# Immortalqx/pi-slam-fusion

Measured on AMD Instinct MI355X. Metric: keyframes/sec fused (4000x3000 -> 256^2 tiles, 5-band), higher is better.
Workload: dtype f32; 1 GPU; cfg-2/cfg-A: 4000x3000 BGR8 keyframes, serpentine sortie, Map2D.Scale=1, 5-band Laplacian, CV_32FC3 (ForceFloat=1) pyramids, frames resident in HBM; frames_per_rank=2646, sortie_frames_before_timing=20, lookahead=48, rendered_rank0=2666, culled_tiles_rank0=490117

## Files before the change

pi-slam-fusion_amd/__init__.py:

```python
import ctypes as C
import os
import subprocess

import numpy as np

_HERE = os.path.dirname(os.path.abspath(__file__))
LIB_PATH = os.environ.get("PF_LIB") or os.path.join(_HERE, "libpifusion.so")
ELE_PIXELS = 256

NoType, TypeCPU, TypeGPU, TypeMultiBandCPU, TypeRender = 0, 1, 2, 3, 4
PF_8UC3, PF_8UC4, PF_16SC3, PF_32FC3 = 16, 24, 19, 21


def host_array(shape, dtype=np.uint8):
    n = int(np.prod(shape)) * np.dtype(dtype).itemsize
    p = lib().pf_host_alloc(n)
    if not p:
        raise MemoryError("pf_host_alloc(%d)" % n)
    buf = (C.c_uint8 * n).from_address(p)
    a = np.frombuffer(buf, dtype=dtype).reshape(shape)
    import weakref
    weakref.finalize(buf, lib().pf_host_free, p)
    return a

# ... 827 lines not shown
    def render_stats(self):
        o = (C.c_double * 4)()
        lib().pf_render_stats(self._h, o)
        return {"frames_with_pixels": int(o[0]), "level0_px": o[1], "owned_px": o[2], "tiles_held": int(o[3])}

    def timers(self):
        cap = 16
        names = (C.c_char_p * cap)(); calls = (C.c_longlong * cap)(); mean = (C.c_double * cap)(); mn = (C.c_double * cap)(); mx = (C.c_double * cap)()
        k = lib().pf_timer_read(self._h, cap, names, calls, mean, mn, mx)
        return {names[i].decode(): {"calls": calls[i], "mean_s": mean[i], "min_s": mn[i], "max_s": mx[i]} for i in range(k)}

    def timer_reset(self):
        lib().pf_timer_reset(self._h)

    def set_cull(self, on):
        lib().pf_set_cull(self._h, 1 if on else 0)

    def next_homography(self, M0):
        if not hasattr(lib(), "pf_debug_next_homography"):
            raise RuntimeError("pf_debug_next_homography: only the experiments library has it (PF_LIB=.../libpifusion_exp.so)")
        a = np.ascontiguousarray(M0, dtype=np.float64).reshape(9)
        lib().pf_debug_next_homography(self._h, a.ctypes.data_as(C.POINTER(C.c_double)))

    def debug_tile_store(self, slab_slots, fail_from=0, fail_count=0):
        if not hasattr(lib(), "pf_debug_tile_store"):
            raise RuntimeError("pf_debug_tile_store: only the experiments library has it (PF_LIB=.../libpifusion_exp.so)")
        lib().pf_debug_tile_store(self._h, int(slab_slots), int(fail_from), int(fail_count))

    def debug_fail_workspace(self, n):
        if not hasattr(lib(), "pf_debug_fail_workspace"):
            raise RuntimeError("pf_debug_fail_workspace: only the experiments library has it (PF_LIB=.../libpifusion_exp.so)")
# ... 24 lines not shown
```

pi-slam-fusion_amd/csrc/c_api.cpp:

```cpp
#include "dist.hpp"
#include "jpeg_device.hpp"
#include "webtiles_plan.hpp"
#include "state_file.hpp"
#include <cerrno>
#include <map>
#include <string>
#include <sys/stat.h>
#include <cstdlib>
#include <cmath>
#include <cstdio>
#include <cstring>
#include <algorithm>
#include <vector>
#include <mutex>
#include <new>

using pf::FusionMap;

struct pf_map {
    FusionMap impl;
    pf::JpegDevice jpeg;
    pf_map(int t, bool th, const pf_options& o) : impl(t, th, o) {}
    ~pf_map() { if (impl.ok() && impl.use_device()) impl.sync(); }
};
// ... 49 lines not shown
}

void pf_destroy(pf_map* m) { delete m; }
const char* pf_last_error(void) { return pf::last_error(); }

int pf_prepare(pf_map* m, const double plane[7], const double cam[6], int n, const pf_image* imgs, const double* poses7)
{ return m && m->impl.prepare(plane, cam, n, imgs, poses7); }

int pf_feed(pf_map* m, const pf_image* img, const double pose[7]) { return m && m->impl.feed(img, pose, false); }
int pf_feed_device(pf_map* m, const pf_image* img, const double pose[7]) { return m && m->impl.feed(img, pose, true); }
int pf_debug_phase_stamps(unsigned long long* out, int cap_blocks) { return pf::read_phase_stamps(out, cap_blocks); }
void pf_debug_form_counts(long long out[8]) { if (out) pf::read_form_counts(out); }
void pf_debug_admission_counts(long long out[8]) { if (out) pf::read_admission_counts(out); }
long long pf_debug_compact_launches(void) { return pf::read_compact_launches(); }
int pf_debug_render_log(pf_map* m, long long* out, int cap) { return m ? m->impl.render_log(out, cap) : 0; }
void pf_set_cull(pf_map* m, int on) { if (m) m->impl.set_cull(on != 0); }
long long pf_debug_culled_cells(pf_map* m) { return m ? m->impl.culled_cells() : 0; }
double pf_debug_level0_exact_px(pf_map* m) { return m ? m->impl.level0_exact_px() : 0; }
long long pf_debug_culled_tiles(pf_map* m) { return m ? m->impl.culled_tiles() : 0; }
int pf_debug_select_counts(unsigned long long* out, int reset) { return out ? pf::read_select_counts(out, reset) : 0; }
long pf_debug_read_last_frame(pf_map* m, void* out, size_t cap) { return m ? m->impl.read_back_last_frame(out, cap) : -1; }
#if PF_EXPERIMENTS
void pf_debug_next_homography(pf_map* m, const double M0[9]) { if (m && M0) m->impl.debug_next_homography(M0); }
void pf_debug_tile_store(pf_map* m, int slab_slots, int fail_from, int fail_count) { if (m) m->impl.debug_tile_store(slab_slots, fail_from, fail_count); }
void pf_debug_fail_workspace(pf_map* m, int n) { if (m) m->impl.debug_fail_workspace(n); }
#endif
unsigned pf_queue_size(pf_map* m) { return m ? m->impl.queue_size() : 0; }
int pf_sync(pf_map* m) { return m && m->impl.sync(); }
int pf_save(pf_map* m, const char* filename) { return m && filename && m->impl.save(filename); }
int pf_save_tiff(pf_map* m, const char* filename, int quality, int force_bigtiff) { return m && filename && m->impl.save_tiff(filename, quality, force_bigtiff != 0); }
int pf_save_tiff_masked(pf_map* m, const char* filename, int quality, int force_bigtiff) { return m && filename && m->impl.save_tiff_masked(filename, quality, force_bigtiff != 0); }
// ... 614 lines not shown
```

pi-slam-fusion_amd/csrc/frame_plan.hpp:

```cpp
#pragma once
#include "plan_limits.hpp"
#include <algorithm>
#include <cmath>
#include <cstdint>
#include <cstring>
#include <vector>

namespace pf {

struct Win { int x0, x1, y0, y1; };


struct CullMargins { double px = 2.0, w = 1e-5; int sub = 4; };

inline bool cull_frame_ok(const double M[9], int crows, int ccols)
{
    const double xs[2] = { -600.0, ccols + 600.0 }, ys[2] = { -600.0, crows + 600.0 };
    int sign = 0;
    for (int i = 0; i < 4; i++) {
        const double x = xs[i & 1], y = ys[i >> 1], W = M[6] * x + M[7] * y + M[8];
        if (!(std::fabs(W) > 1e-12) || !std::isfinite(W)) return false;
        const int sg = W > 0 ? 1 : -1;
        if (sign && sg != sign) return false;
        sign = sg;
// ... 1 lines not shown
    }
    return true;
}

inline float stored_bound(float wlb, bool single_band)
{
    const float gap = single_band ? 3.2f / 254.f : 0.f, floor_w = single_band ? 6.f / 254.f : 0.f;
    return wlb > floor_w ? wlb - gap : 0.f;
}

struct TileCull {
    unsigned out;
    int nraise; int q[16]; float w[16];
};

struct Lattice {
    bool all = false; int nx = 0, ny = 0, dil = 1, cols = 0, rows = 0; double xc = 0, yc = 0, dis_max = 1, inv_dis_max = 1, M[9] = {};
    CullMargins mg;
    std::vector<double> sx, sy, d; std::vector<unsigned char> in;
    std::vector<double> pair_d; std::vector<unsigned char> pair_in; bool paired = false;

    void map_canvas(const double Minv[9], int crows, int ccols, int cols_, int rows_, int dil_, bool map_all, const CullMargins& m)
    {
        all = map_all; mg = m; paired = false;
        dil = dil_;
        nx = ccols / 64 + 2 * dil + 1; ny = crows / 64 + 2 * dil + 1;
        const size_t n = (size_t)nx * ny;
        sx.resize(n); sy.resize(n); d.resize(n); in.assign(n, 2);
        xc = (double)(cols_ / 2); yc = (double)(rows_ / 2); dis_max = std::sqrt(xc * xc + yc * yc);
        inv_dis_max = 1.0 / dis_max;
        cols = cols_; rows = rows_;
        for (int i = 0; i < 9; i++) M[i] = Minv[i];
        if (!map_all) return;
        const double cmax = cols - 2.0, rmax = rows - 2.0;
        for (int m_ = 0; m_ < ny; m_++) {
            const double y = 64.0 * (m_ - dil), n0 = M[1] * y + M[2], n1 = M[4] * y + M[5], w0 = M[7] * y + M[8];
            double* __restrict__ psx = sx.data() + (size_t)m_ * nx; double* __restrict__ psy = sy.data() + (size_t)m_ * nx;
            double* __restrict__ pd = d.data() + (size_t)m_ * nx; unsigned char* __restrict__ pin = in.data() + (size_t)m_ * nx;
            for (int k = 0; k < nx; k++) {
                const double x = 64.0 * (k - dil), iw = 1.0 / (M[6] * x + w0);
                const double px = (M[0] * x + n0) * iw, py = (M[3] * x + n1) * iw, dx = px - xc, dy = py - yc;
                psx[k] = px; psy[k] = py; pd[k] = dx * dx + dy * dy;
            }
            for (int k = 0; k < nx; k++) pin[k] = (unsigned char)((psx[k] >= 1.0) & (psx[k] <= cmax) & (psy[k] >= 1.0) & (psy[k] <= rmax));
        }
    }

    size_t point(int k, int m)
    {
        const size_t o = (size_t)m * nx + k;
        if (in[o] == 2) {
            const double x = 64.0 * (k - dil), y = 64.0 * (m - dil), iw = 1.0 / (M[6] * x + M[7] * y + M[8]);
            const double px = (M[0] * x + M[1] * y + M[2]) * iw, py = (M[3] * x + M[4] * y + M[5]) * iw;
            sx[o] = px; sy[o] = py;
            const double dx = px - xc, dy = py - yc;
            d[o] = dx * dx + dy * dy;
            in[o] = px >= 1.0 && px <= cols - 2.0 && py >= 1.0 && py <= rows - 2.0;
        }
        return o;
    }
// ... 9 lines not shown
            const double far2 = std::max(std::max(d2[0], d2[1]), std::max(d2[2], d2[3]));
            const double tw = weight_type == 0 ? (1.0 - mw - (double)wlb) * dis_max - mpx : 1e300;
            if ((in[c[0]] & in[c[1]] & in[c[2]] & in[c[3]]) == 1 && tw > 0 && far2 < tw * tw * (1.0 + 1e-9)) {
                const double dfar = std::sqrt(far2) + mpx;
                double w = 1.0 - dfar * inv_dis_max;
                if (weight_type != 0) w = w > 0 ? w * w : 0.0;
                w -= mw;
                if (w > 2e-5) *wmin = (float)w;
            }
        }
        if (!want_out || !(wlb > 2e-5f)) return false;
        double g = (double)wlb - mw;
        if (weight_type != 0) g = std::sqrt(g);
        const double T = mpx + dis_max * (1.0 - g), T2 = T * T;
        if (d2[0] <= T2 || d2[1] <= T2 || d2[2] <= T2 || d2[3] <= T2) return false;
        bool pos = true, neg = true; double dnear2 = 1e300;
        for (int i = 0; i < 4; i++) {
            const size_t a = c[i], b = c[(i + 1) & 3];
            const double ex = sx[b] - sx[a], ey = sy[b] - sy[a], px = xc - sx[a], py = yc - sy[a];
            const double cr = ex * py - ey * px;
            pos = pos && cr >= 0; neg = neg && cr <= 0;
            const double e2 = ex * ex + ey * ey, dot = px * ex + py * ey;
            if (dot > 0 && dot < e2) dnear2 = std::min(dnear2, cr * cr / e2);
        }
        if (pos || neg) return false;
        return dnear2 > T2;
    }

    void raise_bounds(int x, int y, int weight_type, float wlb[16])
    {
// ... 47 lines not shown
        if (ask) {
            float wl = wlb[0];
            for (int q = 1; q < S * S; q++) wl = std::min(wl, wlb[q]);
            tile_out = cell_out(4 * x, 4 * y, 4, weight_type, stored_bound(wl, single_band), true, nullptr);
        }
        if (tile_out && pre_raised) c.out = 0xffffu;
        else for (int q = 0; q < S * S; q++) {
            const int qx = q % S, qy = q / S;
            float wmin = 0.f;
            if (cell_out(4 * x + span * qx, 4 * y + span * qy, span, weight_type, stored_bound(wlb[q], single_band), ask && !tile_out, pre_raised ? nullptr : &wmin) || tile_out)
                c.out |= S == 4 ? 1u << q : 0x33u << (8 * qy + 2 * qx);
            if (wmin > wlb[q]) { c.q[c.nraise] = q; c.w[c.nraise++] = wmin; }
        }
        if (fresh && c.out != 0xffffu) c.out = 0;
    }
};

inline void clampw(int lo, int hi, int n, int& o0, int& o1) { o0 = std::max(lo, 0); o1 = std::min(hi, n); }
inline int lv_lo(int p, int i) { return p >> i; }
inline int lv_hi(int p, int i) { return (p + (1 << i) - 1) >> i; }

inline void need_windows(const Win& box, int L, int crows, int ccols, Win N[kMaxLevels])
{
    for (int i = L; i >= 0; i--) {
        int x0 = lv_lo(box.x0, i), x1 = lv_hi(box.x1, i), y0 = lv_lo(box.y0, i), y1 = lv_hi(box.y1, i);
        if (i > 0) { x0 -= 1; x1 += 1; y0 -= 1; y1 += 1; }
        if (i < L) {
            x0 = std::min(x0, 2 * N[i + 1].x0 - 2); x1 = std::max(x1, 2 * N[i + 1].x1 + 1);
            y0 = std::min(y0, 2 * N[i + 1].y0 - 2); y1 = std::max(y1, 2 * N[i + 1].y1 + 1);
        }
        clampw(x0, x1, ccols >> i, N[i].x0, N[i].x1);
        clampw(y0, y1, crows >> i, N[i].y0, N[i].y1);
    }
}

typedef unsigned __int128 u128;
inline u128 col_mask(int x0, int x1) { return (x1 - x0 >= 127 ? ~(u128)0 : (((u128)1 << (x1 - x0 + 1)) - 1)) << x0; }

struct CellList {
    struct Cell { int cx, cy, x0, y0, x1, y1; };
    Cell c[64]; int n = 0; bool overflow = false;
    void add(int cx, int cy, int x0, int y0, int x1, int y1)
    {
        if (overflow) return;
        int k = n - 1;
        while (k >= 0 && !(c[k].cx == cx && c[k].cy == cy)) k--;
        if (k < 0) {
            if (n == 64) overflow = true;
            else c[n++] = Cell{ cx, cy, x0, y0, x1, y1 };
        } else {
            Cell& e = c[k];
            e.x0 = std::min(e.x0, x0); e.y0 = std::min(e.y0, y0); e.x1 = std::max(e.x1, x1); e.y1 = std::max(e.y1, y1);
// ... 174 lines not shown
```

pi-slam-fusion_amd/csrc/fusion_map.cpp:

```cpp
#include "fusion_map.hpp"
#include "map_internal.hpp"
#include "env.hpp"
#include "warp_index.hpp"
#include <algorithm>
#include <cmath>
#include <cstdio>
#include <cstdlib>
#include <cstring>

namespace pf {

FusionMap::FusionMap(int type, bool thread, const pf_options& opt) : opt_(opt), thread_(thread)
{
    single_band_ = (type == PF_TYPE_CPU || type == PF_TYPE_GPU);
    const int lim = (int)std::ceil(std::log((double)kElePixels) / std::log(2.0));
    band_num_ = std::min(opt_.band_number, lim);
    if (band_num_ < 0) band_num_ = 0;
    if (single_band_) band_num_ = 0;
    lay_ = make_layout(band_num_, opt_.force_float != 0);
    if (single_band_) { lay_.f32 = 0; lay_.lap_off[0] = 0; lay_.w_off[0] = 0; lay_.slot_bytes = kElePixels * kElePixels * 4; }
    store_.configure(lay_.slot_bytes);
    if (opt_.max_queue <= 0) opt_.max_queue = 20;
    table_in_args_ = exp_env("PF_TABLE_COPY") == nullptr;
    if (opt_.shard_count < 1) opt_.shard_count = 1;
// ... 159 lines not shown
        p.lat.map_canvas(w.Minv, w.crows, w.ccols, f.cols, f.rows, single_band_ ? 0 : ((2 << w.L) - 2 + 63) / 64, map_all, cull_margins_);
        if (lookahead_ok()) {
            if (!tiles_pool_.empty()) { p.tiles = std::move(tiles_pool_.back()); tiles_pool_.pop_back(); }
            if (!reserve_frame_workspace(w) || !pre_raise(w, p.tiles)) {
                if (p.lat.sx.capacity() && lat_pool_.size() < 8) lat_pool_.push_back(std::move(p.lat));
                if (p.tiles.capacity() && tiles_pool_.size() < 8) tiles_pool_.push_back(std::move(p.tiles));
                pending_.pop_back();
                release_slot(f);
                keyframe_lost();
                return false;
            }
            p.pre_raised = true;
            since_drain_++;
            keep = std::min<size_t>((size_t)opt_.lookahead, 2 * (size_t)since_drain_ / 3);
        }
    }
    while (pending_.size() > keep)
        if (!render_front()) return false;
    return true;
}

bool FusionMap::pre_raise(FrameWork& w, std::vector<Tile*>& tiles)
{
    tiles.assign((size_t)w.tx * w.ty, nullptr);
    const bool sharded = opt_.shard_count > 1;
    for (int y = 0; y < w.ty; y++)
        for (int x = 0; x < w.tx; x++) {
            const int sx = w.xminInt + x + off_x_, sy = w.yminInt + y + off_y_;
            if (sharded && tile_owner(opt_.shard_count, opt_.shard_block, sx, sy) != opt_.shard_rank) continue;
            Tile* t = store_.get_or_create(sx, sy);
// ... 13 lines not shown
    slots_[f.slot].queued = false;
}

bool FusionMap::drain()
{
    since_drain_ = 0;
    if (pending_.empty()) return true;
    if (!set_device()) return false;
    bool ok = true;
    while (!pending_.empty()) ok = render_front() && ok;
    return ok;
}

bool FusionMap::render_front()
{
    const bool ok = render_front_stages();
    if (!ok) keyframe_lost();
    return ok;
}

bool FusionMap::render_front_stages()
{
    struct Pop {
        FusionMap* m;
        ~Pop() {
            PendingFrame& p = m->pending_.front();
            if (p.lat.sx.capacity() && m->lat_pool_.size() < 8) m->lat_pool_.push_back(std::move(p.lat));
            if (p.tiles.capacity() && m->tiles_pool_.size() < 8) m->tiles_pool_.push_back(std::move(p.tiles));
            m->pending_.pop_front();
        }
    } pop{ this };
    PendingFrame& p = pending_.front();
    const QueuedFrame f = p.f;
    struct Held { FusionMap* m; const QueuedFrame& f; bool done = false; ~Held() { if (!done) m->release_slot(f); } } held{ this, f };
    FrameWork& w = fw_;
    w.reset();
    std::memcpy(w.pts, p.pts, sizeof(p.pts));
    w.xminInt = p.sx0 - off_x_; w.yminInt = p.sy0 - off_y_; w.xmaxInt = w.xminInt + p.tx; w.ymaxInt = w.yminInt + p.ty;
    w.tx = p.tx; w.ty = p.ty; w.L = band_num_; w.crows = w.ty * kElePixels; w.ccols = w.tx * kElePixels;
    std::memcpy(w.M0, p.M0, sizeof(p.M0)); std::memcpy(w.Minv, p.Minv, sizeof(p.Minv));
    w.cull = p.cull;
    w.pre_raised = p.pre_raised;
    w.tiles_known = p.tiles.size() == (size_t)p.tx * p.ty ? p.tiles.data() : nullptr;
    if (w.pre_raised && !w.tiles_known) { set_error("render_front: a keyframe admitted without its tiles"); return false; }
    w.src = f.ext ? f.ext : slots_[f.slot].dev;
    w.lat = &p.lat;
    Section sec_apply(this, T_APPLY);
    if (!build_tile_table(f, w)) return false;
    if (w.bx0 >= w.bx1) {
        for (auto& r : w.raise) r.t->wlb[r.q] = std::max(r.t->wlb[r.q], r.w);
        for (Tile* t : w.culled) t->changed = true;
        if (w.owned_all) n_rendered_++;
        log_rendered(f);
        return true;
    }
    px_owned_ += (double)w.owned * kElePixels * kElePixels;
    n_with_pixels_++;
// ... 63 lines not shown
    const bool sharded = w.sharded;
    const bool cull = w.cull;
    const bool lookahead = cull && lookahead_ok();
    if (cull) w.raise.reserve((size_t)tx * ty * cull_margins_.sub * cull_margins_.sub);
    const int B = opt_.shard_block;
    static const int bc_env = exp_env_int("PF_CULL_CELL", 0);
    const int Bc = sharded ? B : (bc_env > 0 ? bc_env : 8);
    table_tmp_.resize((size_t)tx * ty);
    w.touched.reserve((size_t)tx * ty);
    w.bx0 = tx; w.bx1 = 0; w.by0 = ty; w.by1 = 0;
    w.pb = Win{ 1 << 30, 0, 1 << 30, 0 };
    auto add_rect = [&](int sx, int sy, int x0, int y0, int x1, int y1) {
        w.pb.x0 = std::min(w.pb.x0, x0); w.pb.x1 = std::max(w.pb.x1, x1); w.pb.y0 = std::min(w.pb.y0, y0); w.pb.y1 = std::max(w.pb.y1, y1);
        if (sharded || cull) w.cells.add(floordiv(sx, Bc), floordiv(sy, Bc), x0, y0, x1, y1);
    };
    for (int y = 0; y < ty; y++) {
        const int sy = w.yminInt + y + off_y_;
        for (int x = 0; x < tx; x++) {
            const int sx = w.xminInt + x + off_x_;
            uint64_t ent = 0;
            Tile* known = w.tiles_known ? w.tiles_known[(size_t)y * tx + x] : nullptr;
            if (known || ((!sharded || tile_owner(opt_.shard_count, B, sx, sy) == opt_.shard_rank) && !w.tiles_known)) {
                Tile* t = known ? known : store_.get_or_create(sx, sy);
                if (!t) return false;
                w.owned_all++;
                unsigned out = 0;
                if (cull) {
                    TileCull c;
                    w.lat->tile_cull(x, y, t->wlb, t->fresh, lookahead, w.pre_raised, opt_.weight_type, single_band_, c);
                    out = c.out;
                    for (int k = 0; k < c.nraise; k++) w.raise.push_back(FrameWork::Raise{ t, c.q[k], c.w[k] });
                    if (out == 0xffffu && t->fresh) {
                        w.culled_any = true; table_tmp_[(size_t)y * tx + x] = 0; n_culled_tiles_++;
                        continue;
                    }
                    if (out == 0xffffu) {
                        w.culled_any = true; table_tmp_[(size_t)y * tx + x] = 0; n_culled_tiles_++; w.culled.push_back(t);
                        continue;
                    }
                    if (out) { w.culled_any = true; n_culled_cells_ += __builtin_popcount(out); }
                }
                if ((uint64_t)(uintptr_t)t->base >> 48) { set_error("tile slot address above 2^48: the table entry has no room for the cell flags"); return false; }
                ent = (uint64_t)(uintptr_t)t->base | (t->fresh ? 1u : 0u) | ((uint64_t)out << 48);
                w.touched.push_back(t);
                w.owned++;
                w.bx0 = std::min(w.bx0, x); w.bx1 = std::max(w.bx1, x + 1); w.by0 = std::min(w.by0, y); w.by1 = std::max(w.by1, y + 1);
                if (!out) add_rect(sx, sy, x * kElePixels, y * kElePixels, (x + 1) * kElePixels, (y + 1) * kElePixels);
                else
                    for (int r = 0; r < 4; r++) {
                        const unsigned in = ~(out >> (4 * r)) & 15u;
                        if (!in) continue;
                        const int c0 = __builtin_ctz(in), c1 = 32 - __builtin_clz(in);
                        add_rect(sx, sy, x * kElePixels + 64 * c0, y * kElePixels + 64 * r, x * kElePixels + 64 * c1, y * kElePixels + 64 * r + 64);
                    }
            }
            table_tmp_[(size_t)y * tx + x] = ent;
        }
    }
    return true;
}

bool FusionMap::reserve_frame_workspace(FrameWork& w)
{
    const int L = w.L, tx = w.tx, ty = w.ty;
    const size_t es = lay_.f32 ? 4 : 2;
    const bool fused = opt_.fused != 0 && L >= 1;
    const size_t pxb = level_px_bytes(lay_.f32 != 0);
    bool grow = false;
    for (int i = 0; i <= L; i++) {
        const size_t n = (size_t)(w.crows >> i) * (w.ccols >> i);
        if (single_band_) continue;
        if (fused) { if (i >= 1 && i < L && (gw_[i].cap < n * pxb || gw2_[i].cap < n * pxb)) grow = true; }
        else if (g_[i].cap < n * 3 * es || wgt_[i].cap < n * 4) grow = true;
    }
// ... 350 lines not shown
```

pi-slam-fusion_amd/csrc/fusion_map.hpp:

```cpp
#pragma once
#include "../../include/pifusion.h"
#include "geometry.hpp"
#include "kernels.hpp"
#include "map_support.hpp"
#include "dist_plan.hpp"
#include "frame_plan.hpp"
#include "env.hpp"
#include "image_io.hpp"
#include "jpeg_encode.hpp"
#include "tiff_pyramid.hpp"
#include "webtiles.hpp"
#include "merge.hpp"
#include "undistort.hpp"
#include "undistort_plan.hpp"
#include <hip/hip_runtime.h>
#include <condition_variable>
#include <cstdio>
#include <cstdlib>
#include <cstring>
#include <deque>
#include <functional>
#include <mutex>
#include <string>
#include <thread>
// ... 73 lines not shown
    void list_tiles(std::vector<TileRec>& out);
    bool pack_strips(const std::vector<StripReq>& reqs, void* dev_out);
    bool export_tiles(const std::vector<std::pair<int, int>>& tiles, void* dev_out);
    bool blend_tiles(const std::vector<std::pair<int, int>>& tiles, const void* const* halo9, uint8_t* bgr);
    bool reject_mismatched_frame(const pf_image* desc);
    bool frame_needs(const double pose7[7], std::vector<unsigned char>& rank_needs);
    int  stage_frame(const pf_image* desc, bool upload_host, void** dev, size_t* bytes);
    bool feed_staged(int slot, const pf_image* desc, const double pose7[7]);
    void release_staged(int slot) { std::lock_guard<std::mutex> q(qmu_); if (slot >= 0 && slot < (int)slots_.size()) slots_[slot].queued = false; }
    hipStream_t stream() const { return stream_; }
    int  device() const { return device_; }
    bool use_device() { return set_device(); }
    bool single_band() const { return single_band_; }
    bool map_update_inputs(int ix, int iy, double plane7[7], double mn[2], double* ele, int* x, int* y);
    long long culled_tiles() { Drained l(*this); return n_culled_tiles_; }
    void set_cull(bool on) { Drained l(*this); cull_on_ = on; }
    long long culled_cells() { Drained l(*this); return n_culled_cells_; }
    int  render_log(long long* out, int cap);
    double level0_exact_px() const { return px_level0_exact_; }
#if PF_EXPERIMENTS
    void debug_next_homography(const double M0[9]) { std::lock_guard<std::mutex> l(mu_); next_M0_.emplace_back(); std::memcpy(next_M0_.back().m, M0, sizeof(double) * 9); }
    void debug_tile_store(int slab_slots, int fail_from, int fail_count) { std::lock_guard<std::mutex> l(mu_); store_.debug_limits(slab_slots, fail_from, fail_count); }
    void debug_fail_workspace(int n) { std::lock_guard<std::mutex> l(mu_); dbg_fail_workspace_ = n; }
#endif
    bool high_quality() const { return opt_.high_quality_show != 0 && !single_band_; }

    int  num_levels() const { return band_num_ + 1; }
    int  pyramid_type() const { return single_band_ ? PF_8UC4 : (lay_.f32 ? PF_32FC3 : PF_16SC3); }
    bool grid(int dims[4], double geo[6]);
    int  tile_count();
    int  tile_coords(int* xy, int cap);
// ... 110 lines not shown

    struct PipeFrame { bool valid = false; int ring = 0, tx = 0, crows = 0, ccols = 0; Win C[kMaxLevels]; double bytes[kMaxLevels], bytes_run[kMaxLevels];
                       int nrect[kMaxLevels]; BlockRect rect[kMaxLevels][kMaxRects];
                       uint32_t need_bits[kMaxLevels][kNeedWords]; int need_n[kMaxLevels] = {};
                       const uint64_t* table_args = nullptr; int table_n = 0; };
    PipeFrame pipe_[kMaxLevels];
    struct FrameWork {
        double pts[8]; int xminInt, yminInt, xmaxInt, ymaxInt;
        int tx, ty, L, crows, ccols; double M0[9], Minv[9];
        const uint8_t* src;
        bool sharded, cull, culled_any; Lattice* lat;
        bool pre_raised;
        Tile* const* tiles_known;
        struct Raise { Tile* t; int q; float w; };
        std::vector<Raise> raise; std::vector<Tile*> culled, touched;
        CellList cells;
        int bx0, bx1, by0, by1, owned, owned_all;
        Win pb;
        LevelPlan plan;
        int ring; bool table_args; const uint64_t* dtab;
        WarpArgs a;
        void reset() {
            raise.clear(); culled.clear(); touched.clear();
            culled_any = cells.overflow = false; cells.n = 0; owned = owned_all = 0; plan.reset();
            src = nullptr; ring = 0; table_args = false; dtab = nullptr; sharded = cull = pre_raised = false; tiles_known = nullptr; lat = nullptr;
        }
    };
    FrameWork fw_;
    struct PendingFrame {
        QueuedFrame f;
        double pts[8]; int sx0, sy0, tx, ty;
        double M0[9], Minv[9];
        bool cull;
        Lattice lat;
        bool pre_raised = false;
        std::vector<Tile*> tiles;
    };
    std::deque<PendingFrame> pending_;
    unsigned since_drain_ = 0;
    std::vector<Lattice> lat_pool_;
    std::vector<std::vector<Tile*>> tiles_pool_;
    bool lookahead_ok() const { return opt_.lookahead > 0 && (single_band_ || (opt_.fused == 1 && band_num_ >= 1)) && cull_on_; }
    bool render_front();
    bool render_front_stages();
    bool drain();
    void release_slot(const QueuedFrame& f);
    bool pre_raise(FrameWork& w, std::vector<Tile*>& tiles);
    void keyframe_lost() { n_failed_++; fail_pending_ = true; fail_msg_ = last_error(); }
    long long n_failed_ = 0;
    bool fail_pending_ = false;
    std::string fail_msg_;
#if PF_EXPERIMENTS
    int dbg_fail_workspace_ = 0;
#endif
    int  frame_canvas(const QueuedFrame& f, FrameWork& w);
    bool build_tile_table(const QueuedFrame& f, FrameWork& w);
    bool reserve_frame_workspace(FrameWork& w);
    bool place_table(FrameWork& w);
    void warp_args(const QueuedFrame& f, FrameWork& w);
    void plan_fused_levels(FrameWork& w);
    bool launch_single_band(const QueuedFrame& f, FrameWork& w);
    bool launch_fused_pipeline(const QueuedFrame& f, FrameWork& w);
// ... 63 lines not shown
```

pi-slam-fusion_amd/csrc/map_feed.cpp:

```cpp
#include "fusion_map.hpp"
#include "map_internal.hpp"
#include "warp_index.hpp"
#include <cmath>
#include <cstdio>
#include <cstring>
#include <new>

namespace pf {

static void print_frame_mismatch() { std::fprintf(stderr, "MultiBandMap2DCPU::renderFrame: frame.first.cols!=p->_camera.w||frame.first.rows!=p->_camera.h||frame.first.type()!=CV_8UC3\n"); }

bool FusionMap::prepare(const double plane7[7], const double cam[6], int n, const pf_image* imgs, const double* poses7)
{
    if (!init_ok_) { set_error("prepare: no device"); return false; }
    if (n == 0 || !poses7 || cam[0] <= 0 || cam[1] <= 0 || cam[2] == 0 || cam[3] == 0) {
        std::fprintf(stderr, "Map2D::prepare:Not valid prepare!\n");
        return false;
    }
    Camera c{ cam[0], cam[1], cam[2], cam[3], cam[4], cam[5], 1. / cam[2], 1. / cam[3] };
    const Pose plane = pose_from7(plane7), pinv = inverse(plane);
    double mx[3] = { -1e10, -1e10, -1e10 }, mn[3] = { 1e10, 1e10, 1e10 };
    std::vector<Pose> local(n);
    for (int i = 0; i < n; i++) {
        local[i] = mul(pinv, pose_from7(poses7 + 7 * i));
// ... 23 lines not shown
    const int h = (int)std::ceil((mx[1] - mn[1]) / ele_size);
    mx[0] = mn[0] + ele_size * w;
    mx[1] = mn[1] + ele_size * h;

    {
        std::unique_lock<std::mutex> q(qmu_);
        for (auto& f : queue_) if (f.slot >= 0) slots_[f.slot].queued = false;
        queue_.clear();
        idle_cv_.wait(q, [this] { return !worker_busy_; });
    }
    std::lock_guard<std::mutex> l(mu_);
    if (!set_device()) return false;
    if (valid_) (void)drain();
    for (auto& p : pending_) release_slot(p.f);
    pending_.clear();
    HIP_OK(sync_all());
    DevBuf und_table; long long und_uncovered = 0;
    if (und_set_ && !build_undistort_table(und_cam_, c, und_table, &und_uncovered)) return false;
    if (und_set_) { und_table_ = std::move(und_table); und_uncovered_ = und_uncovered; }
    store_.clear();
    plane_ = plane; plane_inv_ = pinv; cam_ = c;
    length_pixel_ = length_pixel; length_pixel_inv_ = 1. / length_pixel;
    ele_size_ = ele_size; ele_size_inv_ = 1. / ele_size;
    std::memcpy(min_, mn, sizeof(mn)); std::memcpy(max_, mx, sizeof(mx)); std::memcpy(min0_, mn, sizeof(mn));
    w_ = w; h_ = h; off_x_ = off_y_ = 0;
    valid_ = true;
    if (thread_ && imgs) {
        for (int i = 0; i < n; i++) {
            if (!imgs[i].data) continue;
            if (frame_mismatch(imgs[i].type, imgs[i].cols, imgs[i].rows)) { print_frame_mismatch(); continue; }
// ... 339 lines not shown
```

pi-slam-fusion_amd/csrc/map_merge.cpp:

```cpp
#include "fusion_map.hpp"
#include "map_internal.hpp"
#include "state_file.hpp"
#include <algorithm>
#include <cmath>
#include <cstdio>
#include <cstring>

namespace pf {

void FusionMap::wait_worker_idle()
{
    if (!thread_) return;
    std::unique_lock<std::mutex> q(qmu_);
    idle_cv_.wait(q, [this] { return queue_.empty() && !worker_busy_; });
}

bool FusionMap::merge_compatible(const char* who, bool single, int pyr, int bands, int weight_type, const double plane7[7], const double cam6[6],
                                 const double min0[3], double ele_size, double length_pixel)
{
    const char* why = nullptr;
    double mine7[7]; std::memcpy(mine7, plane_.t, 24); std::memcpy(mine7 + 3, plane_.q, 32);
    if (single != single_band_) why = "map types differ";
    else if (pyr != pyramid_type()) why = "pyramid types differ";
    else if (bands != band_num_) why = "band numbers differ";
// ... 4 lines not shown
        why = "the maps were prepared differently (tile coordinates are not one frame)";
    if (why) { set_error(std::string(who) + ": " + why); return false; }
    return true;
}

void FusionMap::grow_to(int sx0, int sy0, int sx1, int sy1)
{
    const Win r{ sx0 - off_x_, sx1 - off_x_, sy0 - off_y_, sy1 - off_y_ };
    if (r.x0 < 0 || r.y0 < 0 || r.x1 > w_ || r.y1 > h_) { Section sec(this, T_SPREAD); spread_tiles(r); }
}

bool FusionMap::merge_items(const std::vector<MergeItem>& items)
{
    last_merge_[0] = (double)items.size(); last_merge_[1] = last_merge_[2] = 0; last_merge_[3] = -1; last_merge_[4] = (double)lay_.slot_bytes;
    if (items.empty()) return true;
    size_t missing = 0;
    for (auto& it : items) missing += store_.find(it.ix, it.iy) == nullptr;
    if (missing && !store_.reserve(missing)) return false;
    std::vector<Tile*> tiles(items.size());
    for (size_t i = 0; i < items.size(); i++)
        if (!(tiles[i] = store_.get_or_create(items[i].ix, items[i].iy))) return false;
    if (!settle()) return false;
    std::vector<MergePair> pairs(items.size());
    size_t n_fresh = 0;
    for (size_t i = 0; i < items.size(); i++) {
        pairs[i] = MergePair{ (uint64_t)(uintptr_t)tiles[i]->base, (uint64_t)(uintptr_t)items[i].src, tiles[i]->fresh ? 1u : 0u, 0u };
        n_fresh += tiles[i]->fresh;
    }
    if (!merge_table_.reserve(pairs.size() * sizeof(MergePair))) return false;
    unsigned long long* won = nullptr;
// ... 212 lines not shown
    if ((h.map_type == sf::kTypeSingleBand) != single_band_ || h.pyramid_type != pyramid_type() || h.band_number != band_num_ || h.weight_type != opt_.weight_type) {
        set_error("load_state: the map's options (type, pyramid type, band number, weight type) are not the file's");
        return false;
    }
    {
        std::unique_lock<std::mutex> q(qmu_);
        for (auto& fr : queue_) if (fr.slot >= 0) slots_[fr.slot].queued = false;
        queue_.clear();
        idle_cv_.wait(q, [this] { return !worker_busy_; });
    }
    std::lock_guard<std::mutex> l(mu_);
    if (!set_device()) return false;
    if (valid_) (void)drain();
    for (auto& p : pending_) release_slot(p.f);
    pending_.clear();
    HIP_OK(sync_all());
    store_.clear();
    und_set_ = false; und_table_.release(); und_uncovered_ = 0;
    plane_ = pose_from7(h.plane); plane_inv_ = inverse(plane_);
    cam_ = Camera{ h.cam[0], h.cam[1], h.cam[2], h.cam[3], h.cam[4], h.cam[5], 1. / h.cam[2], 1. / h.cam[3] };
    length_pixel_ = h.length_pixel; length_pixel_inv_ = 1. / h.length_pixel;
    ele_size_ = h.ele_size; ele_size_inv_ = 1. / h.ele_size;
    std::memcpy(min_, h.min, 24); std::memcpy(max_, h.max, 24); std::memcpy(min0_, h.min0, 24);
    w_ = h.w; h_ = h.h; off_x_ = h.off_x; off_y_ = h.off_y;
    valid_ = true;
    return merge_records(f, &h, &heads);
}

}
```

pi-slam-fusion_amd/csrc/map_output.cpp:

```cpp
#include "fusion_map.hpp"
#include "map_internal.hpp"
#include "env.hpp"
#include <algorithm>
#include <cstdlib>
#include <cstring>
#include <thread>

namespace pf {

bool FusionMap::grid(int dims[4], double geo[6])
{
    std::lock_guard<std::mutex> l(mu_);
    if (!valid_) return false;
    dims[0] = w_; dims[1] = h_; dims[2] = off_x_; dims[3] = off_y_;
    geo[0] = min_[0]; geo[1] = min_[1]; geo[2] = max_[0]; geo[3] = max_[1]; geo[4] = ele_size_; geo[5] = length_pixel_;
    return true;
}

bool FusionMap::map_update_inputs(int ix, int iy, double plane7[7], double mn[2], double* ele, int* x, int* y)
{
    Drained l(*this);
    if (!valid_) return false;
    Tile* t = store_.find(ix, iy);
    if (!t || t->fresh) return false;
// ... 63 lines not shown
    Drained l(*this);
    if (!init_ok_ || !set_device()) return false;
    Tile* t = store_.find(ix, iy);
    if (!t || t->fresh) return false;
    HIP_OK(hipMemcpyAsync(dev_out, t->base, lay_.slot_bytes, hipMemcpyDeviceToDevice, stream_));
    HIP_OK(sync_all());
    return true;
}

bool FusionMap::tile_import(int ix, int iy, const void* dev_in)
{
    Drained l(*this);
    if (!init_ok_ || !valid_ || !set_device()) return false;
    Tile* t = store_.get_or_create(ix, iy);
    if (!t) return false;
    HIP_OK(hipMemcpyAsync(t->base, dev_in, lay_.slot_bytes, hipMemcpyDeviceToDevice, stream_));
    HIP_OK(sync_all());
    t->fresh = false; t->changed = true;
    for (float& w : t->wlb) w = -1.f;
    return true;
}

void FusionMap::list_tiles(std::vector<TileRec>& out)
{
    Drained l(*this);
    out.clear();
    store_.for_each([&](int ix, int iy, Tile& t) { if (!t.fresh) out.push_back({ ix, iy, t.changed ? 1 : 0 }); });
    std::sort(out.begin(), out.end(), [](const TileRec& a, const TileRec& b) { return a.iy != b.iy ? a.iy < b.iy : a.ix < b.ix; });
}

// ... 404 lines not shown
```

Measured before the change: 28310 keyframes/s.

## Add pairwise frame-dominance culling and a fast per-cell early accept

```diff
diff --git a/pi-slam-fusion_amd/__init__.py b/pi-slam-fusion_amd/__init__.py
--- a/pi-slam-fusion_amd/__init__.py
+++ b/pi-slam-fusion_amd/__init__.py
@@ -865,7 +865,7 @@
         lib().pf_timer_reset(self._h)
 
     def set_cull(self, on):
-        lib().pf_set_cull(self._h, 1 if on else 0)
+        lib().pf_set_cull(self._h, int(on))
 
     def next_homography(self, M0):
         if not hasattr(lib(), "pf_debug_next_homography"):
diff --git a/pi-slam-fusion_amd/csrc/c_api.cpp b/pi-slam-fusion_amd/csrc/c_api.cpp
--- a/pi-slam-fusion_amd/csrc/c_api.cpp
+++ b/pi-slam-fusion_amd/csrc/c_api.cpp
@@ -87,7 +87,7 @@
 void pf_debug_admission_counts(long long out[8]) { if (out) pf::read_admission_counts(out); }
 long long pf_debug_compact_launches(void) { return pf::read_compact_launches(); }
 int pf_debug_render_log(pf_map* m, long long* out, int cap) { return m ? m->impl.render_log(out, cap) : 0; }
-void pf_set_cull(pf_map* m, int on) { if (m) m->impl.set_cull(on != 0); }
+void pf_set_cull(pf_map* m, int on) { if (m) m->impl.set_cull(on); }
 long long pf_debug_culled_cells(pf_map* m) { return m ? m->impl.culled_cells() : 0; }
 double pf_debug_level0_exact_px(pf_map* m) { return m ? m->impl.level0_exact_px() : 0; }
 long long pf_debug_culled_tiles(pf_map* m) { return m ? m->impl.culled_tiles() : 0; }
diff --git a/pi-slam-fusion_amd/csrc/frame_plan.hpp b/pi-slam-fusion_amd/csrc/frame_plan.hpp
--- a/pi-slam-fusion_amd/csrc/frame_plan.hpp
+++ b/pi-slam-fusion_amd/csrc/frame_plan.hpp
@@ -39,15 +39,31 @@
     int nraise; int q[16]; float w[16];
 };
 
+typedef unsigned __int128 u128;
+inline u128 col_mask(int x0, int x1) { return (x1 - x0 >= 127 ? ~(u128)0 : (((u128)1 << (x1 - x0 + 1)) - 1)) << x0; }
+
+struct PairRecord {
+    long long id = -1;
+    int sx0 = 0, sy0 = 0, tx = 0, ty = 0;
+    double ppx = 0, ppy = 0;
+    double dis_max = 1, px = 2.0, w = 1e-5; int weight_type = 0;
+    double lim2 = 0;
+    std::vector<double> b2;
+    void clear() { id = -1; }
+};
+
 struct Lattice {
     bool all = false; int nx = 0, ny = 0, dil = 1, cols = 0, rows = 0; double xc = 0, yc = 0, dis_max = 1, inv_dis_max = 1, M[9] = {};
     CullMargins mg;
     std::vector<double> sx, sy, d; std::vector<unsigned char> in;
     std::vector<double> pair_d; std::vector<unsigned char> pair_in; bool paired = false;
+    std::vector<double> near2; std::vector<unsigned char> near_rows; bool near_ok = false;
+    double edge2 = 0;
+    std::vector<u128> pr_need, pr_dom; std::vector<double> fr_d;
 
     void map_canvas(const double Minv[9], int crows, int ccols, int cols_, int rows_, int dil_, bool map_all, const CullMargins& m)
     {
-        all = map_all; mg = m; paired = false;
+        all = map_all; mg = m; paired = false; near_ok = false;
         dil = dil_;
         nx = ccols / 64 + 2 * dil + 1; ny = crows / 64 + 2 * dil + 1;
         const size_t n = (size_t)nx * ny;
@@ -56,7 +72,7 @@
         inv_dis_max = 1.0 / dis_max;
         cols = cols_; rows = rows_;
         for (int i = 0; i < 9; i++) M[i] = Minv[i];
-        if (!map_all) return;
+        if (!map_all) { edge2 = cell_edge(); edge2 *= edge2; return; }
         const double cmax = cols - 2.0, rmax = rows - 2.0;
         for (int m_ = 0; m_ < ny; m_++) {
             const double y = 64.0 * (m_ - dil), n0 = M[1] * y + M[2], n1 = M[4] * y + M[5], w0 = M[7] * y + M[8];
@@ -69,6 +85,7 @@
             }
             for (int k = 0; k < nx; k++) pin[k] = (unsigned char)((psx[k] >= 1.0) & (psx[k] <= cmax) & (psy[k] >= 1.0) & (psy[k] <= rmax));
         }
+        edge2 = cell_edge(); edge2 *= edge2;
     }
 
     size_t point(int k, int m)
@@ -108,6 +125,10 @@
         if (weight_type != 0) g = std::sqrt(g);
         const double T = mpx + dis_max * (1.0 - g), T2 = T * T;
         if (d2[0] <= T2 || d2[1] <= T2 || d2[2] <= T2 || d2[3] <= T2) return false;
+        {
+            const double l2 = edge2 * e * e, dmin2 = std::min(std::min(d2[0], d2[1]), std::min(d2[2], d2[3]));
+            if (dmin2 > 4.0 * l2 && dmin2 - 0.25 * l2 > T2) return true;
+        }
         bool pos = true, neg = true; double dnear2 = 1e300;
         for (int i = 0; i < 4; i++) {
             const size_t a = c[i], b = c[(i + 1) & 3];
@@ -185,7 +206,131 @@
         }
         if (fresh && c.out != 0xffffu) c.out = 0;
     }
+
+    int cells_x() const { return nx - 2 * dil - 1; }
+    int cells_y() const { return ny - 2 * dil - 1; }
+
+    double cell_edge()
+    {
+        double pmax = 0, wmin = 1e300;
+        for (int i = 0; i < 4; i++) {
+            const size_t o = point((i & 1) ? nx - 1 : 0, (i >> 1) ? ny - 1 : 0);
+            const double x = 64.0 * (((i & 1) ? nx - 1 : 0) - dil), y = 64.0 * (((i >> 1) ? ny - 1 : 0) - dil);
+            pmax = std::max(pmax, std::sqrt(sx[o] * sx[o] + sy[o] * sy[o]));
+            wmin = std::min(wmin, std::fabs(M[6] * x + M[7] * y + M[8]));
+        }
+        const double lx = std::sqrt(M[0] * M[0] + M[3] * M[3]) + pmax * std::fabs(M[6]), ly = std::sqrt(M[1] * M[1] + M[4] * M[4]) + pmax * std::fabs(M[7]);
+        return 64.0 * std::max(lx, ly) / wmin * (1.0 + 1e-9);
+    }
+
+    void fill_record(PairRecord& r, int weight_type)
+    {
+        const int cw = cells_x(), ch = cells_y();
+        r.tx = cw / 4; r.ty = ch / 4; r.dis_max = dis_max; r.weight_type = weight_type; r.px = mg.px; r.w = mg.w;
+        r.b2.resize((size_t)cw * ch);
+        if (!all)
+            for (int m = dil; m <= dil + ch; m++)
+                for (int k = dil; k <= dil + cw; k++) (void)point(k, m);
+        const double t = weight_type == 0 ? 2e-5 + mg.w : std::sqrt(2e-5 + mg.w), lim = (1.0 - t) * dis_max - mg.px, lim2 = lim > 0 ? lim * lim : 0.0;
+        const double inv2 = inv_dis_max * inv_dis_max, inf = 1e300;
+        r.lim2 = lim2 * inv2;
+        fr_d.resize((size_t)2 * cw + nx);
+        double* __restrict__ md = fr_d.data() + (size_t)2 * cw;
+        for (int m = 0; m <= ch; m++) {
+            const double* __restrict__ dd = d.data() + (size_t)(m + dil) * nx + dil; const unsigned char* __restrict__ ii = in.data() + (size_t)(m + dil) * nx + dil;
+            double* __restrict__ hd = fr_d.data() + (size_t)(m & 1) * cw;
+            for (int cx = 0; cx <= cw; cx++) md[cx] = ii[cx] == 1 ? dd[cx] : inf;
+            for (int cx = 0; cx < cw; cx++) hd[cx] = std::max(md[cx], md[cx + 1]);
+            if (!m) continue;
+            const double* __restrict__ pd = fr_d.data() + (size_t)(~m & 1) * cw;
+            double* __restrict__ b2 = r.b2.data() + (size_t)(m - 1) * cw;
+            for (int cx = 0; cx < cw; cx++) b2[cx] = std::max(hd[cx], pd[cx]) * inv2;
+        }
+    }
+
+    const double* near_row(int cy)
+    {
+        const int cw = cells_x();
+        double* __restrict__ a2 = near2.data() + (size_t)cy * cw;
+        if (!near_rows[(size_t)cy]) {
+            near_rows[(size_t)cy] = 1;
+            if (!all) for (int m = cy + dil; m <= cy + dil + 1; m++) for (int k = dil; k <= dil + cw; k++) (void)point(k, m);
+            const double* __restrict__ d0 = d.data() + (size_t)(cy + dil) * nx + dil; const double* __restrict__ d1 = d0 + nx;
+            const double l2 = edge2, inv2 = inv_dis_max * inv_dis_max;
+            for (int cx = 0; cx < cw; cx++) {
+                const double dmin2 = std::min(std::min(d0[cx], d0[cx + 1]), std::min(d1[cx], d1[cx + 1]));
+                a2[cx] = dmin2 > 4.0 * l2 ? (dmin2 - 0.25 * l2) * inv2 : 0.0;
+            }
+        }
+        return a2;
+    }
+
+    void pair_out(int sx0, int sy0, int weight_type, const PairRecord& g, const u128* want, u128* out)
+    {
+        const int cw = cells_x(), ch = cells_y(), e = dil;
+        if (g.id < 0 || cw > 128 || g.weight_type != weight_type || g.px != mg.px || g.w != mg.w || g.b2.size() != (size_t)16 * g.tx * g.ty) return;
+        const int ox = 4 * (g.sx0 - sx0), oy = 4 * (g.sy0 - sy0);
+        const int x0 = std::max(0, ox), x1 = std::min(cw, ox + 4 * g.tx), y0 = std::max(0, oy), y1 = std::min(ch, oy + 4 * g.ty);
+        if (x1 - x0 < 2 * e + 1 || y1 - y0 < 2 * e + 1) return;
+        const double c = mg.px * inv_dis_max + mg.px / g.dis_max + (weight_type == 0 ? 2.0 * mg.w : std::sqrt(2.0 * mg.w));
+        if (!(c < 0.5)) return;
+        const double inv = 1.0 / (1.0 - c), blim = g.lim2;
+        const u128 inner = col_mask(x0 + e, x1 - e - 1);
+        pr_need.assign((size_t)ch, 0); pr_dom.assign((size_t)ch, 0);
+        bool any = false;
+        for (int r = y0 + e; r < y1 - e; r++) {
+            const u128 m = want[r] & inner;
+            if (!m) continue;
+            any = true;
+            u128 dm = m;
+            for (int s = 1; s <= e; s++) dm |= (m << s) | (m >> s);
+            for (int rr = r - e; rr <= r + e; rr++) pr_need[(size_t)rr] |= dm;
+        }
+        if (!any) return;
+        if (!near_ok) { near2.resize((size_t)cw * ch); near_rows.assign((size_t)ch, 0); near_ok = true; }
+        const int gw = 4 * g.tx;
+        for (int r = y0; r < y1; r++) {
+            const u128 need = pr_need[(size_t)r];
+            if (!need) continue;
+            const uint64_t lo64 = (uint64_t)need, hi64 = (uint64_t)(need >> 64);
+            const int lo = lo64 ? __builtin_ctzll(lo64) : 64 + __builtin_ctzll(hi64), hi = hi64 ? 127 - __builtin_clzll(hi64) : 63 - __builtin_clzll(lo64);
+            const double* __restrict__ a2 = near_row(r);
+            const double* __restrict__ b2 = g.b2.data() + (size_t)(r - oy) * gw;
+            unsigned char flag[136];
+            const int n = hi - lo + 1;
+            for (int j = 0; j < n; j++) flag[j] = (unsigned char)((a2[lo + j] > b2[lo + j - ox] * inv + c) & (b2[lo + j - ox] < blim));
+            std::memset(flag + n, 0, 8);
+            u128 dom = 0;
+            for (int j = 0; j < n; j += 8) {
+                uint64_t x;
+                std::memcpy(&x, flag + j, 8);
+                dom |= (u128)((x * 0x0102040810204080ull) >> 56) << j;
+            }
+            pr_dom[(size_t)r] = (dom << lo) & need;
+        }
+        for (int r = y0 + e; r < y1 - e; r++) {
+            u128 m = want[r] & inner;
+            for (int rr = r - e; rr <= r + e && m; rr++) {
+                const u128 dd = pr_dom[(size_t)rr];
+                u128 h = dd;
+                for (int s = 1; s <= e; s++) h &= (dd << s) & (dd >> s);
+                m &= h;
+            }
+            out[r] |= m;
+        }
+    }
 };
+
+inline unsigned rows_tile_bits(const u128* rows, int x, int y)
+{
+    unsigned b = 0;
+    for (int r = 0; r < 4; r++) b |= ((unsigned)(rows[4 * y + r] >> (4 * x)) & 15u) << (4 * r);
+    return b;
+}
+inline void tile_bits_rows(u128* rows, int x, int y, unsigned bits)
+{
+    for (int r = 0; r < 4; r++) rows[4 * y + r] |= (u128)((bits >> (4 * r)) & 15u) << (4 * x);
+}
 
 inline void clampw(int lo, int hi, int n, int& o0, int& o1) { o0 = std::max(lo, 0); o1 = std::min(hi, n); }
 inline int lv_lo(int p, int i) { return p >> i; }
@@ -204,9 +349,6 @@
         clampw(y0, y1, crows >> i, N[i].y0, N[i].y1);
     }
 }
-
-typedef unsigned __int128 u128;
-inline u128 col_mask(int x0, int x1) { return (x1 - x0 >= 127 ? ~(u128)0 : (((u128)1 << (x1 - x0 + 1)) - 1)) << x0; }
 
 struct CellList {
     struct Cell { int cx, cy, x0, y0, x1, y1; };
diff --git a/pi-slam-fusion_amd/csrc/fusion_map.cpp b/pi-slam-fusion_amd/csrc/fusion_map.cpp
--- a/pi-slam-fusion_amd/csrc/fusion_map.cpp
+++ b/pi-slam-fusion_amd/csrc/fusion_map.cpp
@@ -197,6 +197,15 @@
             since_drain_++;
             keep = std::min<size_t>((size_t)opt_.lookahead, 2 * (size_t)since_drain_ / 3);
         }
+        if (pair_on() && !single_band_) {
+            PairRecord& r = pair_ring_[(size_t)pair_next_];
+            pair_next_ = (pair_next_ + 1) % kPairRing;
+            r.id = p.pair_id = ++pair_seq_;
+            r.sx0 = p.sx0; r.sy0 = p.sy0;
+            const double cx = (double)(f.cols / 2), cy = (double)(f.rows / 2), iw = 1.0 / (w.M0[6] * cx + w.M0[7] * cy + w.M0[8]);
+            r.ppx = (w.M0[0] * cx + w.M0[1] * cy + w.M0[2]) * iw; r.ppy = (w.M0[3] * cx + w.M0[4] * cy + w.M0[5]) * iw;
+            p.lat.fill_record(r, opt_.weight_type);
+        }
     }
     while (pending_.size() > keep)
         if (!render_front()) return false;
@@ -240,8 +249,9 @@
 
 bool FusionMap::render_front()
 {
+    const long long id = pending_.front().pair_id;
     const bool ok = render_front_stages();
-    if (!ok) keyframe_lost();
+    if (!ok) { keyframe_lost(); pair_forget(id); }
     return ok;
 }
 
@@ -267,6 +277,7 @@
     std::memcpy(w.M0, p.M0, sizeof(p.M0)); std::memcpy(w.Minv, p.Minv, sizeof(p.Minv));
     w.cull = p.cull;
     w.pre_raised = p.pre_raised;
+    w.pair_id = p.pair_id;
     w.tiles_known = p.tiles.size() == (size_t)p.tx * p.ty ? p.tiles.data() : nullptr;
     if (w.pre_raised && !w.tiles_known) { set_error("render_front: a keyframe admitted without its tiles"); return false; }
     w.src = f.ext ? f.ext : slots_[f.slot].dev;
@@ -360,22 +371,34 @@
         w.pb.x0 = std::min(w.pb.x0, x0); w.pb.x1 = std::max(w.pb.x1, x1); w.pb.y0 = std::min(w.pb.y0, y0); w.pb.y1 = std::max(w.pb.y1, y1);
         if (sharded || cull) w.cells.add(floordiv(sx, Bc), floordiv(sy, Bc), x0, y0, x1, y1);
     };
+    w.tl.assign((size_t)tx * ty, nullptr); w.outs.assign((size_t)tx * ty, 0);
+    for (int y = 0; y < ty; y++) {
+        const int sy = w.yminInt + y + off_y_;
+        for (int x = 0; x < tx; x++) {
+            const int sx = w.xminInt + x + off_x_;
+            Tile* known = w.tiles_known ? w.tiles_known[(size_t)y * tx + x] : nullptr;
+            if (!(known || ((!sharded || tile_owner(opt_.shard_count, B, sx, sy) == opt_.shard_rank) && !w.tiles_known))) continue;
+            Tile* t = known ? known : store_.get_or_create(sx, sy);
+            if (!t) return false;
+            w.tl[(size_t)y * tx + x] = t;
+            if (cull) {
+                TileCull c;
+                w.lat->tile_cull(x, y, t->wlb, t->fresh, lookahead, w.pre_raised, opt_.weight_type, single_band_, c);
+                w.outs[(size_t)y * tx + x] = c.out;
+                for (int k = 0; k < c.nraise; k++) w.raise.push_back(FrameWork::Raise{ t, c.q[k], c.w[k] });
+            }
+        }
+    }
+    if (cull && !single_band_ && pair_on() && w.pair_id >= 0 && 4 * tx <= 128) pair_cull(w);
     for (int y = 0; y < ty; y++) {
         const int sy = w.yminInt + y + off_y_;
         for (int x = 0; x < tx; x++) {
             const int sx = w.xminInt + x + off_x_;
             uint64_t ent = 0;
-            Tile* known = w.tiles_known ? w.tiles_known[(size_t)y * tx + x] : nullptr;
-            if (known || ((!sharded || tile_owner(opt_.shard_count, B, sx, sy) == opt_.shard_rank) && !w.tiles_known)) {
-                Tile* t = known ? known : store_.get_or_create(sx, sy);
-                if (!t) return false;
+            if (Tile* t = w.tl[(size_t)y * tx + x]) {
                 w.owned_all++;
-                unsigned out = 0;
+                const unsigned out = w.outs[(size_t)y * tx + x];
                 if (cull) {
-                    TileCull c;
-                    w.lat->tile_cull(x, y, t->wlb, t->fresh, lookahead, w.pre_raised, opt_.weight_type, single_band_, c);
-                    out = c.out;
-                    for (int k = 0; k < c.nraise; k++) w.raise.push_back(FrameWork::Raise{ t, c.q[k], c.w[k] });
                     if (out == 0xffffu && t->fresh) {
                         w.culled_any = true; table_tmp_[(size_t)y * tx + x] = 0; n_culled_tiles_++;
                         continue;
@@ -404,6 +427,52 @@
         }
     }
     return true;
+}
+
+void FusionMap::pair_cull(FrameWork& w)
+{
+    const int tx = w.tx, ty = w.ty;
+    const bool lookahead = lookahead_ok();
+    w.want.assign((size_t)4 * ty, 0); w.pout.assign((size_t)4 * ty, 0);
+    bool any = false;
+    for (int y = 0; y < ty; y++)
+        for (int x = 0; x < tx; x++) {
+            Tile* t = w.tl[(size_t)y * tx + x];
+            if (!t || (t->fresh && !lookahead)) continue;
+            const unsigned in = ~w.outs[(size_t)y * tx + x] & 0xffffu;
+            if (in) { tile_bits_rows(w.want.data(), x, y, in); any = true; }
+        }
+    if (!any) return;
+    const int sx0 = w.xminInt + off_x_, sy0 = w.yminInt + off_y_;
+    static const int n_cand = std::min(std::max(exp_env_int("PF_CULL_PAIR_N", 2), 1), kPairCandidates);
+    const PairRecord* cand[kPairCandidates]; double cd[kPairCandidates]; int nc = 0;
+    const PairRecord* self = nullptr;
+    for (const PairRecord& r : pair_ring_) if (r.id == w.pair_id) self = &r;
+    if (!self) return;
+    for (const PairRecord& r : pair_ring_) {
+        if (r.id < 0 || r.id == w.pair_id) continue;
+        if (r.sx0 >= sx0 + tx || r.sx0 + r.tx <= sx0 || r.sy0 >= sy0 + ty || r.sy0 + r.ty <= sy0) continue;
+        const double dx = (256.0 * r.sx0 + r.ppx) - (256.0 * sx0 + self->ppx), dy = (256.0 * r.sy0 + r.ppy) - (256.0 * sy0 + self->ppy);
+        const double d2 = dx * dx + dy * dy;
+        if (nc == n_cand) { if (d2 >= cd[nc - 1]) continue; nc--; }
+        int k = nc++;
+        while (k > 0 && cd[k - 1] > d2) { cand[k] = cand[k - 1]; cd[k] = cd[k - 1]; k--; }
+        cand[k] = &r; cd[k] = d2;
+    }
+    for (int i = 0; i < nc; i++) {
+        w.lat->pair_out(sx0, sy0, opt_.weight_type, *cand[i], w.want.data(), w.pout.data());
+        for (size_t r = 0; r < w.want.size(); r++) w.want[r] &= ~w.pout[r];
+    }
+    for (int y = 0; y < ty; y++)
+        for (int x = 0; x < tx; x++) {
+            Tile* t = w.tl[(size_t)y * tx + x];
+            if (!t) continue;
+            const unsigned add = rows_tile_bits(w.pout.data(), x, y);
+            if (!add) continue;
+            unsigned& out = w.outs[(size_t)y * tx + x];
+            if (t->fresh && (out | add) != 0xffffu) continue;
+            out |= add;
+        }
 }
 
 bool FusionMap::reserve_frame_workspace(FrameWork& w)
diff --git a/pi-slam-fusion_amd/csrc/fusion_map.hpp b/pi-slam-fusion_amd/csrc/fusion_map.hpp
--- a/pi-slam-fusion_amd/csrc/fusion_map.hpp
+++ b/pi-slam-fusion_amd/csrc/fusion_map.hpp
@@ -111,7 +111,7 @@
     bool single_band() const { return single_band_; }
     bool map_update_inputs(int ix, int iy, double plane7[7], double mn[2], double* ele, int* x, int* y);
     long long culled_tiles() { Drained l(*this); return n_culled_tiles_; }
-    void set_cull(bool on) { Drained l(*this); cull_on_ = on; }
+    void set_cull(int on) { Drained l(*this); cull_on_ = on != 0; pair_always_ = on == 2; pair_clear(); }
     long long culled_cells() { Drained l(*this); return n_culled_cells_; }
     int  render_log(long long* out, int cap);
     double level0_exact_px() const { return px_level0_exact_; }
@@ -252,6 +252,8 @@
         Tile* const* tiles_known;
         struct Raise { Tile* t; int q; float w; };
         std::vector<Raise> raise; std::vector<Tile*> culled, touched;
+        std::vector<Tile*> tl; std::vector<unsigned> outs;
+        long long pair_id; std::vector<u128> want, pout;
         CellList cells;
         int bx0, bx1, by0, by1, owned, owned_all;
         Win pb;
@@ -261,7 +263,7 @@
         void reset() {
             raise.clear(); culled.clear(); touched.clear();
             culled_any = cells.overflow = false; cells.n = 0; owned = owned_all = 0; plan.reset();
-            src = nullptr; ring = 0; table_args = false; dtab = nullptr; sharded = cull = pre_raised = false; tiles_known = nullptr; lat = nullptr;
+            src = nullptr; ring = 0; table_args = false; dtab = nullptr; sharded = cull = pre_raised = false; tiles_known = nullptr; lat = nullptr; pair_id = -1;
         }
     };
     FrameWork fw_;
@@ -272,6 +274,7 @@
         bool cull;
         Lattice lat;
         bool pre_raised = false;
+        long long pair_id = -1;
         std::vector<Tile*> tiles;
     };
     std::deque<PendingFrame> pending_;
@@ -284,6 +287,15 @@
     bool drain();
     void release_slot(const QueuedFrame& f);
     bool pre_raise(FrameWork& w, std::vector<Tile*>& tiles);
+    static constexpr int kPairRing = 64, kPairCandidates = 8;
+    std::vector<PairRecord> pair_ring_ = std::vector<PairRecord>(kPairRing);
+    int pair_next_ = 0; long long pair_seq_ = 0;
+    int  pair_env_ = exp_env_int("PF_CULL_PAIR", -1);
+    bool pair_always_ = false;
+    bool pair_on() const { return pair_env_ >= 0 ? pair_env_ != 0 : (pair_always_ || !lookahead_ok()); }
+    void pair_clear() { for (PairRecord& r : pair_ring_) r.clear(); }
+    void pair_forget(long long id) { if (id >= 0) for (PairRecord& r : pair_ring_) if (r.id == id) r.clear(); }
+    void pair_cull(FrameWork& w);
     void keyframe_lost() { n_failed_++; fail_pending_ = true; fail_msg_ = last_error(); }
     long long n_failed_ = 0;
     bool fail_pending_ = false;
diff --git a/pi-slam-fusion_amd/csrc/map_feed.cpp b/pi-slam-fusion_amd/csrc/map_feed.cpp
--- a/pi-slam-fusion_amd/csrc/map_feed.cpp
+++ b/pi-slam-fusion_amd/csrc/map_feed.cpp
@@ -61,6 +61,7 @@
     if (valid_) (void)drain();
     for (auto& p : pending_) release_slot(p.f);
     pending_.clear();
+    pair_clear();
     HIP_OK(sync_all());
     DevBuf und_table; long long und_uncovered = 0;
     if (und_set_ && !build_undistort_table(und_cam_, c, und_table, &und_uncovered)) return false;
diff --git a/pi-slam-fusion_amd/csrc/map_merge.cpp b/pi-slam-fusion_amd/csrc/map_merge.cpp
--- a/pi-slam-fusion_amd/csrc/map_merge.cpp
+++ b/pi-slam-fusion_amd/csrc/map_merge.cpp
@@ -42,6 +42,7 @@
 {
     last_merge_[0] = (double)items.size(); last_merge_[1] = last_merge_[2] = 0; last_merge_[3] = -1; last_merge_[4] = (double)lay_.slot_bytes;
     if (items.empty()) return true;
+    pair_clear();
     size_t missing = 0;
     for (auto& it : items) missing += store_.find(it.ix, it.iy) == nullptr;
     if (missing && !store_.reserve(missing)) return false;
@@ -284,6 +285,7 @@
     if (valid_) (void)drain();
     for (auto& p : pending_) release_slot(p.f);
     pending_.clear();
+    pair_clear();
     HIP_OK(sync_all());
     store_.clear();
     und_set_ = false; und_table_.release(); und_uncovered_ = 0;
diff --git a/pi-slam-fusion_amd/csrc/map_output.cpp b/pi-slam-fusion_amd/csrc/map_output.cpp
--- a/pi-slam-fusion_amd/csrc/map_output.cpp
+++ b/pi-slam-fusion_amd/csrc/map_output.cpp
@@ -101,6 +101,7 @@
     if (!init_ok_ || !valid_ || !set_device()) return false;
     Tile* t = store_.get_or_create(ix, iy);
     if (!t) return false;
+    pair_clear();
     HIP_OK(hipMemcpyAsync(t->base, dev_in, lay_.slot_bytes, hipMemcpyDeviceToDevice, stream_));
     HIP_OK(sync_all());
     t->fresh = false; t->changed = true;
```

Result: slower. 27950 keyframes/s (-1.3%).
